# nekopanda/Amatsukaze

Measured on NVIDIA B200. Metric: 1920x1080i YV12 frames/sec (logo-eval + combing), higher is better.
Workload: dtype u8+f32

## Files before the change

### amatsukaze_b200/csrc/amtk_b200.cu

```cuda
#include "amtk_internal.h"
#include "logo_kernels.cuh"
#include "comb_kernels.cuh"
#include "comb_stream.cuh"
#include "comb_mma.cuh"
#include "scan_kernels.cuh"
#include <algorithm>
#include <cfloat>
#include <cmath>
#include <cstdlib>
#include <cstring>
#include <mutex>

extern "C" { static int logo_ensure_device(const amtk_logo* cl, amtk_ctx* ctx, bool need_tables); }

namespace amtk {

static thread_local std::string g_error;
static constexpr size_t kEvalSmemLimit = 226 * 1024;
void set_error(const std::string& msg) { g_error = msg; }
bool cuda_ok(cudaError_t e, const char* what) {
  if (e == cudaSuccess) return true;
  set_error(std::string("CUDA error: ") + cudaGetErrorString(e) + " in " + what);
  return false;
}
// ... 263 lines not shown
}

static bool roi_inside(const amtk::HostLogo& full, const amtk_clip* clip, int pitch_elems) {
  if (full.imgx < 0 || full.imgy < 0) return false;
  const long long last = (long long)full.imgx + full.w - 1 + (long long)(full.imgy + full.h - 1) * pitch_elems;
  const long long plane_elems = (long long)clip->pitch_y / clip->bytes_per_sample * clip->height;
  return full.imgx + full.w <= pitch_elems && last < plane_elems;
}

static int comb_thresholds_ok(const amtk_comb_params* p, int bytes_per_sample) {
  if (bytes_per_sample == 2) {
    const int all[6] = { p->th_move_y, p->th_shima_y, p->th_lshima_y, p->th_move_c, p->th_shima_c, p->th_lshima_c };
    for (int v : all) if (v < 1) { set_error("comb: thresholds must be >= 1"); return 0; }
    if (p->th_move_y > 32768 || p->th_move_c > 32768) { set_error("comb: th_move must be in [1,32768] for 16-bit samples"); return 0; }
    return 1;
  }
  const int m[2] = { p->th_move_y, p->th_move_c };
  const int s[4] = { p->th_shima_y, p->th_lshima_y, p->th_shima_c, p->th_lshima_c };
  for (int v : m) if (v < 1 || v > 128) { set_error("comb: th_move must be in [1,128]"); return 0; }
  for (int v : s) if (v < 1 || v > 2047) { set_error("comb: th_shima/th_lshima must be in [1,2047]"); return 0; }
  return 1;
}

struct CombVariant {
  int R, strip, stages, sync, TH, boxH, threads, smem;
  void (*kernel)(const CombArgs);
  void (*kernel16)(const CombArgs);
};
template <typename Cfg> static CombVariant make_variant() {
  return CombVariant{ Cfg::R, Cfg::STRIP, Cfg::STAGES, Cfg::SYNC, Cfg::TH, Cfg::BOXH, Cfg::THREADS, Cfg::SMEM, comb_tma_kernel<Cfg, 1>, nullptr };
}
template <typename Cfg> static CombVariant make_variant16() {
  return CombVariant{ Cfg::R, Cfg::STRIP, Cfg::STAGES, Cfg::SYNC, Cfg::TH, Cfg::BOXH, Cfg::THREADS, Cfg::SMEM, comb_tma_kernel<Cfg, 1>, comb_tma_kernel<Cfg, 2> };
}
static const CombVariant* comb_variants(int* n) {
  static const CombVariant v[] = {
    make_variant16<CombCfg<15, 8, 3, 0>>(), make_variant16<CombCfg<16, 8, 3, 0>>(), make_variant16<CombCfg<17, 8, 3, 0>>(),
    make_variant<CombCfg<17, 8, 2, 0>>(), make_variant<CombCfg<17, 8, 4, 0>>(), make_variant<CombCfg<17, 8, 3, 1>>(),
  };
  *n = (int)(sizeof(v) / sizeof(v[0]));
  return v;
}

static int pick_comb_R(int hY, int hC) {
  int best = 16; long long best_waste = -1;
  for (int R = 17; R >= 15; --R) {
    const int th = 8 * R;
    const long long waste = (long long)((hY + th - 1) / th) * th - hY + 2LL * (((hC + th - 1) / th) * th - hC) / 2;
    if (best_waste < 0 || waste < best_waste) { best_waste = waste; best = R; }
  }
  return best;
}

struct WsVariant { int R, stages, warps, bps, TH, boxH, smem; void (*kernel)(const WsArgs); };
template <typename Cfg> static WsVariant make_ws() { return WsVariant{ Cfg::R, Cfg::STAGES, Cfg::WARPS, Cfg::BPS, Cfg::TH, Cfg::BOXH, Cfg::SMEM, comb_ws_kernel<Cfg> }; }
static const WsVariant* ws_variants(int* n) {
  static const WsVariant v[] = { make_ws<WsCfg<17, 2>>(), make_ws<WsCfg<15, 2>>(), make_ws<WsCfg<16, 2>>(), make_ws<WsCfg<9, 2>>(), make_ws<WsCfg<15, 3>>(), make_ws<WsCfg<12, 2>>(), make_ws<WsCfg<10, 2>>(),
                                 make_ws<WsCfg<15, 2, 7>>(), make_ws<WsCfg<13, 2, 5>>(), make_ws<WsCfg<15, 2, 2>>(), make_ws<WsCfg<15, 3, 3>>(),
                                 make_ws<WsCfg<15, 2, 4, 2>>(), make_ws<WsCfg<16, 2, 4, 2>>(), make_ws<WsCfg<17, 2, 4, 2>>() };
  *n = (int)(sizeof(v) / sizeof(v[0]));
  return v;
}
static int pick_ws_R(int hY, int hC) {
  int best = 17; long long best_waste = -1;
  for (int R : { 17, 16, 15 }) {
    const int th = 4 * R;
    const long long waste = 2LL * ((long long)((hY + th - 1) / th) * th - hY) + 2LL * ((long long)((hC + th - 1) / th) * th - hC);
    if (best_waste < 0 || waste < best_waste) { best_waste = waste; best = R; }
  }
  return best;
}

static int launch_comb_ws(amtk_ctx* ctx, const amtk_clip* clip, const Window& win, int lo, int hi,
                          const amtk_comb_params* prm, int* dcounts, int out_row0) {
  const int hY = clip->height, hC = clip->height >> clip->log_uvy;
  const int wY = clip->width, wC = clip->width >> clip->log_uvx;
  const int R = ctx->knobs.comb_R ? ctx->knobs.comb_R : pick_ws_R(hY, hC);
  int nvar = 0; const WsVariant* vars = ws_variants(&nvar); const WsVariant* V = nullptr;
  const int bps = clip->bytes_per_sample;
  for (int i = 0; i < nvar; ++i) if (vars[i].R == R && vars[i].stages == ctx->knobs.comb_ws_stages && vars[i].warps == ctx->knobs.comb_ws_warps && vars[i].bps == bps) V = &vars[i];
  if (!V) AMTK_FAIL("comb: no warp-stream kernel variant for the requested AMTK_COMB_* settings");
  const int WW = V->warps;
  WsArgs args;
  memset(&args, 0, sizeof(args));
  const CUtensorMapL2promotion promo = ctx->knobs.comb_l2 == 0 ? CU_TENSOR_MAP_L2_PROMOTION_NONE : ctx->knobs.comb_l2 == 64 ? CU_TENSOR_MAP_L2_PROMOTION_L2_64B :
                                       ctx->knobs.comb_l2 == 256 ? CU_TENSOR_MAP_L2_PROMOTION_L2_256B : CU_TENSOR_MAP_L2_PROMOTION_L2_128B;
  for (int pl = 0; pl < 3; ++pl) {
    const long long off = pl == 0 ? 0 : (pl == 1 ? clip->off_u : clip->off_v);
    cuuint64_t gdim[3] = { (cuuint64_t)(pl ? wC : wY) * bps, (cuuint64_t)(pl ? hC : hY), (cuuint64_t)win.count };
    cuuint64_t gstr[2] = { (cuuint64_t)(pl ? clip->pitch_uv : clip->pitch_y), (cuuint64_t)clip->frame_stride };
    cuuint32_t box[3] = { (cuuint32_t)kWsTW, (cuuint32_t)V->boxH, 1u };
    cuuint32_t estr[3] = { 1u, 1u, 1u };
    if (ctx->encode_tiled(&args.map[pl], CU_TENSOR_MAP_DATA_TYPE_UINT8, 3, const_cast<uint8_t*>(win.dev_base) + off, gdim, gstr, box, estr,
                          CU_TENSOR_MAP_INTERLEAVE_NONE, CU_TENSOR_MAP_SWIZZLE_NONE, promo, CU_TENSOR_MAP_FLOAT_OOB_FILL_NONE) != CUDA_SUCCESS)
      AMTK_FAIL("cuTensorMapEncodeTiled failed");
  }
  const int remC = (wC * bps) % kWsTW;
  const long long uv_dist = clip->off_v - clip->off_u;
  const bool pair_uv = ctx->knobs.comb_merge_uv && remC > 0 && remC <= kWsTW / 2 && uv_dist > 0 && (uv_dist & 15) == 0;
  if (pair_uv) {
    cuuint64_t gdim[4] = { (cuuint64_t)wC * bps, 2u, (cuuint64_t)hC, (cuuint64_t)win.count };
    cuuint64_t gstr[3] = { (cuuint64_t)uv_dist, (cuuint64_t)clip->pitch_uv, (cuuint64_t)clip->frame_stride };
    cuuint32_t box[4] = { (cuuint32_t)(kWsTW / 2), 2u, (cuuint32_t)V->boxH, 1u };
    cuuint32_t estr[4] = { 1u, 1u, 1u, 1u };
    if (ctx->encode_tiled(&args.map_uv, CU_TENSOR_MAP_DATA_TYPE_UINT8, 4, const_cast<uint8_t*>(win.dev_base) + clip->off_u, gdim, gstr, box, estr,
                          CU_TENSOR_MAP_INTERLEAVE_NONE, CU_TENSOR_MAP_SWIZZLE_NONE, promo, CU_TENSOR_MAP_FLOAT_OOB_FILL_NONE) != CUDA_SUCCESS)
      AMTK_FAIL("cuTensorMapEncodeTiled(uv pair) failed");
  }
  const int tyY = (hY + V->TH - 1) / V->TH, tyC = (hC + V->TH - 1) / V->TH;
  int tile0 = 0, nc = 0;
  auto thresholds = [&](WsClass& C, bool chroma) {
    C.cls = chroma ? 1 : 0; C.H = chroma ? hC : hY;
    const int tM = chroma ? prm->th_move_c : prm->th_move_y, tS = chroma ? prm->th_shima_c : prm->th_shima_y, tL = chroma ? prm->th_lshima_c : prm->th_lshima_y;
    if (bps == 1) {
      C.thM = (unsigned)(0x80 - tM) * 0x01010101u;
      C.thS = (unsigned)tS * 0x00010001u;
      C.thL = (unsigned)tL * 0x00010001u;
    } else {
      C.thM = (unsigned)std::min(tM, 2047) * 0x00010001u;
      C.thS = (unsigned)(8192 + std::min(tS, 8191)) * 0x00010001u;
      C.thL = (unsigned)(8192 + std::min(tL, 8191)) * 0x00010001u;
    }
  };
  for (int pl = 0; pl < 3; ++pl) {
    WsClass& C = args.cl[nc];
    const int w = (pl ? wC : wY) * bps;
    C.kind = 0; C.map = pl; thresholds(C, pl != 0);
    C.tilesX = (pl && pair_uv) ? w / kWsTW : (w + kWsTW - 1) / kWsTW;
    C.tile0 = tile0; C.ntiles = C.tilesX * (pl ? tyC : tyY);
    if (C.ntiles == 0) continue;
    tile0 += C.ntiles; ++nc;
  }
  if (pair_uv) {
    WsClass& C = args.cl[nc];
    C.kind = 1; C.x0 = wC * bps - remC; C.tilesX = 1; thresholds(C, true);
    C.tile0 = tile0; C.ntiles = tyC; tile0 += C.ntiles; ++nc;
  }
  args.nclasses = nc;
  const int ntiles = tile0, nf = hi - lo;
  amtk_ctx::CombPlan& plan = ctx->plan;
  if (plan.occ_kernel != (const void*)V->kernel) {
    int occ = 0;
    AMTK_CUDA(cudaFuncSetAttribute(V->kernel, cudaFuncAttributeMaxDynamicSharedMemorySize, V->smem));
    AMTK_CUDA(cudaOccupancyMaxActiveBlocksPerMultiprocessor(&occ, V->kernel, 32 * WW, V->smem));
    if (occ < 1) AMTK_FAIL("comb kernel does not fit on an SM");
    plan.occ = occ; plan.occ_kernel = (const void*)V->kernel; plan.valid = false;
  }
  int occ = plan.occ;
  if (ctx->knobs.comb_ctas > 0) occ = std::min(occ, ctx->knobs.comb_ctas);
  const long long total = (long long)ntiles * nf;
  const int nwarps = ctx->sm_count * occ * WW;
  const int grid = (int)std::min<long long>((long long)ctx->sm_count * occ, (total + WW - 1) / WW);
  const int f0 = lo - win.first;
  if (!(plan.valid && plan.wY == wY && plan.hY == hY && plan.wC == wC && plan.hC == hC && plan.nf == nf && plan.f0 == f0 &&
        plan.R == V->R + 100 * bps && plan.item == ctx->knobs.comb_item + 1000 * ctx->knobs.comb_tail && plan.ctas == occ * WW)) {
    int big = ctx->knobs.comb_item > 0 ? ctx->knobs.comb_item : 64, small = std::max(4, big / 4);
    while (big > 8 && (long long)ntiles * (nf / big) < 6LL * nwarps) { big /= 2; small = std::max(4, big / 4); }
    const int tail_frames = std::min(nf, std::max(small, (int)(nf * 0.15)));
    const int head_frames = nf - tail_frames;
    const int tiny = ctx->knobs.comb_tail;
    const int end_frames = (tiny > 0 && tiny < small) ? std::min(tail_frames, std::max(tiny, (int)(nf * 0.04))) : 0;
    const int mid_end = nf - end_frames;
    std::vector<CombSegment> segs;
    segs.reserve((size_t)ntiles * (head_frames / big + tail_frames / small + (tiny > 0 ? end_frames / tiny : 0) + 3));
    for (int t = 0; t < ntiles; ++t)
      for (int f = 0; f < head_frames; f += big) segs.push_back(CombSegment{ t, f0 + f, f0 + std::min(head_frames, f + big) });
    for (int t = 0; t < ntiles; ++t)
      for (int f = head_frames; f < mid_end; f += small) segs.push_back(CombSegment{ t, f0 + f, f0 + std::min(mid_end, f + small) });
    for (int t = 0; t < ntiles; ++t)
      for (int f = mid_end; f < nf; f += tiny) segs.push_back(CombSegment{ t, f0 + f, f0 + std::min(nf, f + tiny) });
    const size_t seg_bytes = segs.size() * sizeof(CombSegment);
    plan.q_off = (seg_bytes + 255) & ~(size_t)255;
    plan.valid = false;
    if (!ensure(&plan.dev, &plan.cap, plan.q_off + 256)) return 0;
    AMTK_CUDA(cudaMemcpyAsync(plan.dev, segs.data(), seg_bytes, cudaMemcpyHostToDevice, ctx->stream));
    AMTK_CUDA(cudaStreamSynchronize(ctx->stream));
    plan.nitems = (int)segs.size();
    plan.wY = wY; plan.hY = hY; plan.wC = wC; plan.hC = hC; plan.nf = nf; plan.f0 = f0; plan.R = V->R + 100 * bps;
    plan.item = ctx->knobs.comb_item + 1000 * ctx->knobs.comb_tail; plan.ctas = occ * WW; plan.valid = true;
  }
  AMTK_CUDA(cudaMemsetAsync(reinterpret_cast<uint8_t*>(plan.dev) + plan.q_off, 0, 256, ctx->stream));
  args.segs = reinterpret_cast<const CombSegment*>(plan.dev);
  args.nitems = plan.nitems;
  args.queue = reinterpret_cast<int*>(reinterpret_cast<uint8_t*>(plan.dev) + plan.q_off);
  args.counts = dcounts;
  args.out_frame0 = out_row0 - win.first;
  AMTK_CUDA(cudaMemsetAsync(dcounts + (size_t)(lo - out_row0) * 12, 0, (size_t)nf * 12 * sizeof(int), ctx->stream));
  std::pair<cudaEvent_t, cudaEvent_t> ev{ nullptr, nullptr };
  if (ctx->timing) {
    if (!ctx->timing_pool.empty()) { ev = ctx->timing_pool.back(); ctx->timing_pool.pop_back(); }
    else { AMTK_CUDA(cudaEventCreate(&ev.first)); AMTK_CUDA(cudaEventCreate(&ev.second)); }
    AMTK_CUDA(cudaEventRecord(ev.first, ctx->stream));
  }
  args.prefetch = ctx->knobs.comb_ws_prefetch;
  if (ctx->want_side_mark) {
    AMTK_CUDA(cudaEventRecord(ctx->ev_side, ctx->stream));
    ctx->want_side_mark = false;
  }
  V->kernel<<<grid, 32 * WW, V->smem, ctx->stream>>>(args);
  AMTK_CUDA(cudaGetLastError());
  if (ctx->timing) { AMTK_CUDA(cudaEventRecord(ev.second, ctx->stream)); ctx->timing_events.push_back(ev); }
  ctx->launches += 1;
  return 1;
}

static int launch_comb_mma(amtk_ctx* ctx, const amtk_clip* clip, const Window& win, int lo, int hi,
                           const amtk_comb_params* prm, int* dcounts, int out_row0) {
  const int hY = clip->height, hC = clip->height >> clip->log_uvy;
  const int wY = clip->width, wC = clip->width >> clip->log_uvx;
  WsArgs args;
  memset(&args, 0, sizeof(args));
  const CUtensorMapL2promotion promo = ctx->knobs.comb_l2 == 0 ? CU_TENSOR_MAP_L2_PROMOTION_NONE : ctx->knobs.comb_l2 == 64 ? CU_TENSOR_MAP_L2_PROMOTION_L2_64B :
                                       ctx->knobs.comb_l2 == 256 ? CU_TENSOR_MAP_L2_PROMOTION_L2_256B : CU_TENSOR_MAP_L2_PROMOTION_L2_128B;
  for (int pl = 0; pl < 3; ++pl) {
    const long long off = pl == 0 ? 0 : (pl == 1 ? clip->off_u : clip->off_v);
    cuuint64_t gdim[3] = { (cuuint64_t)(pl ? wC : wY), (cuuint64_t)(pl ? hC : hY), (cuuint64_t)win.count };
    cuuint64_t gstr[2] = { (cuuint64_t)(pl ? clip->pitch_uv : clip->pitch_y), (cuuint64_t)clip->frame_stride };
    cuuint32_t box[3] = { (cuuint32_t)kMmTW, (cuuint32_t)kMmBoxH, 1u };
    cuuint32_t estr[3] = { 1u, 1u, 1u };
    if (ctx->encode_tiled(&args.map[pl], CU_TENSOR_MAP_DATA_TYPE_UINT8, 3, const_cast<uint8_t*>(win.dev_base) + off, gdim, gstr, box, estr,
                          CU_TENSOR_MAP_INTERLEAVE_NONE, CU_TENSOR_MAP_SWIZZLE_128B, promo, CU_TENSOR_MAP_FLOAT_OOB_FILL_NONE) != CUDA_SUCCESS)
      AMTK_FAIL("cuTensorMapEncodeTiled failed");
  }
  const int tyY = (hY + kMmTH - 1) / kMmTH, tyC = (hC + kMmTH - 1) / kMmTH;
  int tile0 = 0, nc = 0;
  for (int pl = 0; pl < 3; ++pl) {
    WsClass& C = args.cl[nc];
    const bool chroma = pl != 0;
    C.kind = 0; C.map = pl; C.cls = chroma ? 1 : 0; C.H = chroma ? hC : hY;
    C.thM = (unsigned)(0x80 - (chroma ? prm->th_move_c : prm->th_move_y)) * 0x01010101u;
    C.thS = (unsigned)(chroma ? prm->th_shima_c : prm->th_shima_y) * 0x00010001u;
// ... 244 lines not shown
  *out = nullptr;
  int n = 0;
  if (cudaGetDeviceCount(&n) != cudaSuccess || n == 0) { cudaGetLastError(); AMTK_FAIL("no CUDA device: this library has no CPU fallback"); }
  if (device < 0 || device >= n) AMTK_FAIL("amtk_ctx_create: bad device ordinal");
  int prev = 0; AMTK_CUDA(cudaGetDevice(&prev));
  AMTK_CUDA(cudaSetDevice(device));
  cudaDeviceProp prop; AMTK_CUDA(cudaGetDeviceProperties(&prop, device));
  if (prop.major != 10) { cudaSetDevice(prev); AMTK_FAIL("this build targets sm_100a (Blackwell B200) only"); }
  amtk_ctx* c = new amtk_ctx();
  c->device = device; c->sm_count = prop.multiProcessorCount;
  c->stream = reinterpret_cast<cudaStream_t>(cuda_stream); c->own_stream = false;
  bool ok = cuda_ok(cudaStreamCreateWithFlags(&c->copy_stream, cudaStreamNonBlocking), "cudaStreamCreate(copy)") &&
            cuda_ok(cudaStreamCreateWithFlags(&c->side_stream, cudaStreamNonBlocking), "cudaStreamCreate(side)") &&
            cuda_ok(cudaEventCreateWithFlags(&c->ev_side, cudaEventDisableTiming), "cudaEventCreate") &&
            cuda_ok(cudaEventCreateWithFlags(&c->ev_side_done, cudaEventDisableTiming), "cudaEventCreate") &&
            cuda_ok(cudaStreamCreateWithFlags(&c->side_stream2, cudaStreamNonBlocking), "cudaStreamCreate(side2)") &&
            cuda_ok(cudaEventCreateWithFlags(&c->ev_fork, cudaEventDisableTiming), "cudaEventCreate") &&
            cuda_ok(cudaEventCreateWithFlags(&c->ev_join1, cudaEventDisableTiming), "cudaEventCreate") &&
            cuda_ok(cudaEventCreateWithFlags(&c->ev_join2, cudaEventDisableTiming), "cudaEventCreate");
  for (int b = 0; b < 2 && ok; ++b) {
    ok = cuda_ok(cudaEventCreateWithFlags(&c->ev_copy[b], cudaEventDisableTiming), "cudaEventCreate") &&
         cuda_ok(cudaEventCreateWithFlags(&c->ev_done[b], cudaEventDisableTiming), "cudaEventCreate");
  }
  std::call_once(g_driver_once, [] {
    void* fn = nullptr; cudaDriverEntryPointQueryResult q;
    if (cudaGetDriverEntryPoint("cuTensorMapEncodeTiled", &fn, cudaEnableDefault, &q) == cudaSuccess && q == cudaDriverEntryPointSuccess)
      g_encode = reinterpret_cast<amtk_encode_tiled_fn>(fn);
    else cudaGetLastError();
  });
  c->encode_tiled = g_encode;
  if (const char* e = getenv("AMTK_COMB_STRIP")) c->knobs.comb_strip = atoi(e);
  if (const char* e = getenv("AMTK_COMB_STAGES")) c->knobs.comb_stages = atoi(e);
  if (const char* e = getenv("AMTK_COMB_R")) c->knobs.comb_R = atoi(e);
  if (const char* e = getenv("AMTK_COMB_CTAS")) c->knobs.comb_ctas = atoi(e);
  if (const char* e = getenv("AMTK_COMB_SYNC")) c->knobs.comb_sync = atoi(e);
  if (const char* e = getenv("AMTK_COMB_GENERIC")) c->knobs.comb_generic = atoi(e);
  if (const char* e = getenv("AMTK_COMB_MERGE_UV")) c->knobs.comb_merge_uv = atoi(e);
  if (const char* e = getenv("AMTK_COMB_PART")) c->knobs.comb_part = atoi(e);
  if (const char* e = getenv("AMTK_EVAL_WAVES")) c->knobs.eval_waves = std::max(1, atoi(e));
  if (const char* e = getenv("AMTK_COMB_L2")) c->knobs.comb_l2 = atoi(e);
  if (const char* e = getenv("AMTK_COMB_WS")) c->knobs.comb_ws = atoi(e);
  if (const char* e = getenv("AMTK_SCAN_LITE")) c->knobs.scan_lite = atoi(e);
  if (const char* e = getenv("AMTK_LITE_CTAS")) c->knobs.lite_ctas = std::max(1, atoi(e));
  if (const char* e = getenv("AMTK_COMB_WS_STAGES")) c->knobs.comb_ws_stages = atoi(e);
  if (const char* e = getenv("AMTK_COMB_ITEM")) c->knobs.comb_item = atoi(e);
  if (const char* e = getenv("AMTK_COMB_TAIL")) c->knobs.comb_tail = atoi(e);
  if (const char* e = getenv("AMTK_COMB_MMA")) c->knobs.comb_mma = atoi(e);
  if (const char* e = getenv("AMTK_COMB_WS10")) c->knobs.comb_ws10 = atoi(e);
  if (const char* e = getenv("AMTK_EVAL_CW")) c->knobs.eval_cw = atoi(e);
  if (const char* e = getenv("AMTK_EVAL_PAR")) c->knobs.eval_par = atoi(e);
  if (const char* e = getenv("AMTK_SCAN_OVERLAP")) c->knobs.scan_overlap = atoi(e);
  if (const char* e = getenv("AMTK_COMB_WS_WARPS")) c->knobs.comb_ws_warps = atoi(e);
  if (const char* e = getenv("AMTK_COMB_WS_PF")) c->knobs.comb_ws_prefetch = atoi(e);
  cudaSetDevice(prev);
  if (!ok) { amtk_ctx_destroy(c); return 0; }
  *out = c;
  return 1;
}

void amtk_ctx_destroy(amtk_ctx* c) {
  if (!c) return;
  int prev = 0; cudaGetDevice(&prev); cudaSetDevice(c->device);
  if (c->stream) cudaStreamSynchronize(c->stream);
  if (c->copy_stream) { cudaStreamSynchronize(c->copy_stream); cudaStreamDestroy(c->copy_stream); }
  if (c->side_stream) { cudaStreamSynchronize(c->side_stream); cudaStreamDestroy(c->side_stream); }
  if (c->ev_side) cudaEventDestroy(c->ev_side);
  if (c->ev_side_done) cudaEventDestroy(c->ev_side_done);
  if (c->side_stream2) { cudaStreamSynchronize(c->side_stream2); cudaStreamDestroy(c->side_stream2); }
  for (cudaEvent_t e : { c->ev_fork, c->ev_join1, c->ev_join2 }) if (e) cudaEventDestroy(e);
  for (int b = 0; b < 2; ++b) { if (c->ev_copy[b]) cudaEventDestroy(c->ev_copy[b]); if (c->ev_done[b]) cudaEventDestroy(c->ev_done[b]); if (c->stage[b]) cudaFree(c->stage[b]); }
  if (c->scratch) cudaFree(c->scratch);
  if (c->small) cudaFree(c->small);
  if (c->dout) cudaFree(c->dout);
  if (c->dout2) cudaFree(c->dout2);
  if (c->hout) cudaFreeHost(c->hout);
  if (c->plan.dev) cudaFree(c->plan.dev);
  for (auto* v : { &c->timing_events, &c->timing_pool }) for (auto& ev : *v) { cudaEventDestroy(ev.first); cudaEventDestroy(ev.second); }
  if (c->own_stream && c->stream) cudaStreamDestroy(c->stream);
  cudaSetDevice(prev);
  delete c;
}

int amtk_ctx_synchronize(amtk_ctx* c) {
  if (!c) AMTK_FAIL("null context");
  DevSelect ds(c); if (!ds.ok) return 0;
  AMTK_CUDA(cudaStreamSynchronize(c->stream));
  return 1;
}
int64_t amtk_ctx_launch_count(const amtk_ctx* c) { return c ? c->launches : 0; }
int64_t amtk_ctx_last_h2d_bytes(const amtk_ctx* c) { return c ? c->h2d_bytes_last : 0; }

int amtk_ctx_set_kernel_timing(amtk_ctx* c, int enable) {
  if (!c) AMTK_FAIL("null context");
  c->timing = enable != 0;
  return 1;
}

int amtk_ctx_get_kernel_timing(amtk_ctx* c, double* ms_total, int64_t* launches, int reset) {
  if (!c) AMTK_FAIL("null context");
  DevSelect ds(c); if (!ds.ok) return 0;
  AMTK_CUDA(cudaStreamSynchronize(c->stream));
  for (auto& ev : c->timing_events) {
    float ms = 0.0f;
    AMTK_CUDA(cudaEventElapsedTime(&ms, ev.first, ev.second));
    c->timing_ms += ms; c->timing_count += 1;
    c->timing_pool.push_back(ev);
// ... 728 lines not shown
```

### amatsukaze_b200/csrc/amtk_internal.h

```cpp
#pragma once
#include <cuda.h>
#include <cuda_runtime.h>
#include <cstdint>
#include <cstdio>
#include <mutex>
#include <string>
#include <vector>
#include "../../include/amtk_b200.h"
#include "logo_host.h"

typedef CUresult (*amtk_encode_tiled_fn)(CUtensorMap*, CUtensorMapDataType, cuuint32_t, void*, const cuuint64_t*,
                                         const cuuint64_t*, const cuuint32_t*, const cuuint32_t*, CUtensorMapInterleave,
                                         CUtensorMapSwizzle, CUtensorMapL2promotion, CUtensorMapFloatOOBfill);

namespace amtk {

void set_error(const std::string& msg);
bool cuda_ok(cudaError_t e, const char* what);

#define AMTK_CUDA(call)                                          \
  do {                                                           \
    if (!::amtk::cuda_ok((call), #call)) return 0;               \
  } while (0)
#define AMTK_FAIL(msg)                                           \
// ... 5 lines not shown
struct LogoDev {
  int w, h, count, countPad;
  float blackScore;
  const float* A;
  const float* B;
  const uint32_t* pix;
  const float* tapsT;
  const float2* scales;
};

}

struct amtk_ctx {
  mutable std::recursive_mutex mu;
  int device = 0;
  cudaStream_t stream = nullptr;
  bool own_stream = false;
  cudaStream_t copy_stream = nullptr;
  cudaStream_t side_stream = nullptr;
  cudaEvent_t ev_side = nullptr, ev_side_done = nullptr;
  cudaStream_t side_stream2 = nullptr;
  cudaEvent_t ev_fork = nullptr, ev_join1 = nullptr, ev_join2 = nullptr;
  size_t scratch_off = 0;
  cudaEvent_t ev_copy[2] = { nullptr, nullptr };
  cudaEvent_t ev_done[2] = { nullptr, nullptr };
  int sm_count = 0;
  int64_t launches = 0;
  long long h2d_bytes_last = 0;
  void* scratch = nullptr; size_t scratch_bytes = 0;
  void* stage[2] = { nullptr, nullptr }; size_t stage_bytes = 0;
  void* small = nullptr; size_t small_bytes = 0;
  void* dout = nullptr; size_t dout_bytes = 0;
  void* dout2 = nullptr; size_t dout2_bytes = 0;
  std::vector<std::pair<const void*, int>> smem_attr;
  void* hout = nullptr; void* hout_dev = nullptr;
  amtk_encode_tiled_fn encode_tiled = nullptr;
  bool want_side_mark = false;
  struct Knobs {
    int eval_waves = 1;
    int eval_cw = 1;
    int eval_par = 1;
    int scan_overlap = 0;
    int comb_generic = 0;
    int comb_merge_uv = 1;
    int comb_part = -1;
    int comb_strip = 8, comb_stages = 3, comb_R = 0, comb_ctas = 0, comb_sync = 0, comb_l2 = 64;
    int comb_item = 0;
    int comb_tail = 4;
    int comb_ws_stages = 2;
    int comb_mma = 0;
    int comb_ws10 = 1;
    int comb_ws_warps = 4;
    int comb_ws_prefetch = 0;
    int lite_ctas = 5;
    int scan_lite = 0;
    int comb_ws = 1;
  } knobs;
  struct CombPlan {
    bool valid = false;
    int wY = 0, hY = 0, wC = 0, hC = 0, nf = 0, f0 = 0, R = 0, item = 0, ctas = 0;
    void* dev = nullptr; size_t cap = 0;
    int nitems = 0; size_t q_off = 0;
    int occ = 0; const void* occ_kernel = nullptr;
  } plan;
  bool timing = false;
  std::vector<std::pair<cudaEvent_t, cudaEvent_t>> timing_events;
  std::vector<std::pair<cudaEvent_t, cudaEvent_t>> timing_pool;
  double timing_ms = 0.0; int64_t timing_count = 0;
};

struct amtk_logo {
  int device = -1;
  amtk::HostLogo host;
  float* dA = nullptr; float* dB = nullptr;
  float* dAU = nullptr; float* dBU = nullptr; float* dAV = nullptr; float* dBV = nullptr;
  uint32_t* dPix = nullptr; float* dTapsT = nullptr; float2* dScales = nullptr;
  int countPad = 0;
  bool has_mask = false;
  bool tables_uploaded = false;
  std::mutex mu;
};

struct amtk_scan {
  amtk_ctx* ctx = nullptr;
  int device = 0;
  int scanw = 0, scanh = 0, logUVx = 1, logUVy = 1, thy = 0;
  int nvalid = 0;
  unsigned long long* dSums = nullptr;
  unsigned long long* dBg = nullptr;
  size_t npix = 0;
};
```

### amatsukaze_b200/csrc/comb_stream.cuh

```cuda
#pragma once
#include <cuda_fp16.h>
#include "amtk_internal.h"
#include "tma_utils.cuh"
#include "comb_kernels.cuh"

namespace amtk {

constexpr int kWsTW = 128;
constexpr int kWsRuns = 4;
constexpr int kWsWarps = 4;

template <int R_, int STAGES_, int WARPS_ = kWsWarps, int BPS_ = 1>
struct WsCfg {
  static constexpr int R = R_, STAGES = STAGES_, WARPS = WARPS_;
  static constexpr int BPS = BPS_;
  static constexpr int TH = kWsRuns * R;
  static constexpr int BOXH = TH + 4;
  static constexpr int STAGE_BYTES = kWsTW * BOXH;
  static constexpr int RING_BYTES = STAGES * STAGE_BYTES;
  static constexpr int SMEM = WARPS * RING_BYTES + 128;
  static constexpr int FIT = (227 * 1024) / (SMEM + 1024 + 8 * WARPS * STAGES + 8);
  static constexpr int MIN_CTAS = FIT >= 4 ? 4 : FIT >= 3 ? 3 : FIT >= 2 ? 2 : 1;
};

struct WsClass {
  int tile0, ntiles;
  int kind;
  int tilesX;
  int map;
  int x0;
  int H;
  int cls;
  unsigned thM, thS, thL;
};
constexpr int kWsMaxClasses = 4;
struct WsArgs {
  CUtensorMap map[3];
  CUtensorMap map_uv;
  WsClass cl[kWsMaxClasses];
  int nclasses;
  const CombSegment* segs;
  int nitems;
  int* queue;
  int* counts;
  int out_frame0;
  int prefetch;
};

__device__ __forceinline__ void tma_load_4d(void* smem_dst, const CUtensorMap* map, uint64_t* bar, int c0, int c1, int c2, int c3) {
  asm volatile(
      "cp.async.bulk.tensor.4d.shared::cluster.global.mbarrier::complete_tx::bytes [%0], [%1, {%3, %4, %5, %6}], [%2];"
      ::"r"(smem_u32(smem_dst)), "l"(map), "r"(smem_u32(bar)), "r"(c0), "r"(c1), "r"(c2), "r"(c3)
      : "memory");
}

__device__ __forceinline__ void tma_prefetch_3d(const CUtensorMap* map, int c0, int c1, int c2) {
  asm volatile("cp.async.bulk.prefetch.tensor.3d.L2.global.tile [%0, {%1, %2, %3}];" ::"l"(map), "r"(c0), "r"(c1), "r"(c2) : "memory");
}
__device__ __forceinline__ void tma_prefetch_4d(const CUtensorMap* map, int c0, int c1, int c2, int c3) {
  asm volatile("cp.async.bulk.prefetch.tensor.4d.L2.global.tile [%0, {%1, %2, %3, %4}];" ::"l"(map), "r"(c0), "r"(c1), "r"(c2), "r"(c3) : "memory");
}

#ifndef AMTK_WS_RELOAD_PREV
#define AMTK_WS_RELOAD_PREV 1
#endif
constexpr bool kWsReloadPrev = AMTK_WS_RELOAD_PREV != 0;
#ifndef AMTK_WS_L_VIA_IDP
#define AMTK_WS_L_VIA_IDP 0
#endif
// ... 167 lines not shown
  W4 h2 = w4(*reinterpret_cast<const uint4*>(cur + 2 * PITCH));
  W4 h3 = w4(*reinterpret_cast<const uint4*>(cur + 3 * PITCH));
#pragma unroll
  for (int j = 0; j < R; ++j) {
    const W4 h4 = w4(*reinterpret_cast<const uint4*>(cur + (j + 4) * PITCH));
    const W4 pv = w4(P[j]);
    const int f = j & 1;
    uint32_t mM[4];
#pragma unroll
    for (int q = 0; q < 4; ++q)
      mM[q] = __hge2_mask(__habs2(__hsub2(*reinterpret_cast<const __half2*>(&h2.v[q]), *reinterpret_cast<const __half2*>(&pv.v[q]))), thM);
    c.M[f] = c.M[f] - (mM[0] + mM[1]) - (mM[2] + mM[3]);
    if (kWsReloadPrev) P[j] = lds128(cur + (j + 2) * PITCH); else P[j] = make_uint4(h2.v[0], h2.v[1], h2.v[2], h2.v[3]);
    ws_row_masks10(h0, h1, h2, h3, h4, thS, thL, c.S[f], c.L[f]);
    h0 = h1; h1 = h2; h2 = h3; h3 = h4;
  }
  return c;
}

template <int PITCH>
__device__ __noinline__ void ws_fixup10(const uint8_t* cur, uint32_t rows, uint32_t mine, uint32_t thS_bits, uint32_t thL_bits, WsCounts& c) {
  const __half2 thS = *reinterpret_cast<const __half2*>(&thS_bits);
  const __half2 thL = *reinterpret_cast<const __half2*>(&thL_bits);
  for (uint32_t m = rows; m; m &= m - 1) {
    const int j = __ffs(m) - 1;
    if (!((mine >> j) & 1u)) continue;
    const uint8_t* p = cur + j * PITCH;
    uint32_t dS = 0u, dL = 0u;
    ws_row_masks10(w4(*reinterpret_cast<const uint4*>(p)), w4(*reinterpret_cast<const uint4*>(p + PITCH)), w4(*reinterpret_cast<const uint4*>(p + 2 * PITCH)),
                   w4(*reinterpret_cast<const uint4*>(p + 3 * PITCH)), w4(*reinterpret_cast<const uint4*>(p + 4 * PITCH)), thS, thL, dS, dL);
    c.S[j & 1] -= dS; c.L[j & 1] -= dL;
  }
}

template <int PITCH>
__device__ __noinline__ void ws_fixup(const uint8_t* cur, uint32_t rows, uint32_t mine, uint32_t thS_bits, uint32_t thL_bits, WsCounts& c) {
  const __half2 thS = *reinterpret_cast<const __half2*>(&thS_bits);
  const __half2 thL = *reinterpret_cast<const __half2*>(&thL_bits);
  for (uint32_t m = rows; m; m &= m - 1) {
    const int j = __ffs(m) - 1;
    if (!((mine >> j) & 1u)) continue;
    const uint8_t* p = cur + j * PITCH;
    const H8 h0 = bytes16_to_half(*reinterpret_cast<const uint4*>(p));
    const H8 h1 = bytes16_to_half(*reinterpret_cast<const uint4*>(p + PITCH));
    const H8 h2 = bytes16_to_half(*reinterpret_cast<const uint4*>(p + 2 * PITCH));
    const H8 h3 = bytes16_to_half(*reinterpret_cast<const uint4*>(p + 3 * PITCH));
    const H8 h4 = bytes16_to_half(*reinterpret_cast<const uint4*>(p + 4 * PITCH));
    uint32_t dS = 0u, dL = 0u;
    ws_row_masks(h0, h1, h2, h3, h4, thS, thL, dS, dL);
    c.S[j & 1] -= dS; c.L[j & 1] -= dL;
  }
}

template <typename Cfg>
__global__ void __launch_bounds__(32 * Cfg::WARPS, Cfg::MIN_CTAS) comb_ws_kernel(const __grid_constant__ WsArgs a) {
  constexpr int S = Cfg::STAGES, R = Cfg::R;
  extern __shared__ uint8_t smem_raw[];
  __shared__ __align__(8) uint64_t full_bars[Cfg::WARPS][S];
  const int lane = threadIdx.x & 31, warp = threadIdx.x >> 5;
  uint8_t* tiles = smem_raw + ((128u - (smem_u32(smem_raw) & 127u)) & 127u) + warp * Cfg::RING_BYTES;
  uint64_t* full_bar = full_bars[warp];
  if (lane == 0) {
#pragma unroll
    for (int s = 0; s < S; ++s) mbar_init(&full_bar[s], 1);
    asm volatile("fence.mbarrier_init.release.cluster;" ::: "memory");
  }
  __syncwarp();
  uint32_t gload = 0;
  const int strip = lane & 7, run = lane >> 3;
  const int lane_off = (run * R) * kWsTW + strip * 16;
  for (;;) {
    int item = 0;
    if (lane == 0) item = atomicAdd(a.queue, 1);
    item = __shfl_sync(0xFFFFFFFFu, item, 0);
    if (item >= a.nitems) break;
    const CombSegment seg = a.segs[item];
    int ci = 0;
#pragma unroll
    for (int k = 1; k < kWsMaxClasses; ++k) if (k < a.nclasses && seg.tile >= a.cl[k].tile0) ci = k;
    const WsClass& C = a.cl[ci];
    const int lt = seg.tile - C.tile0;
    const int ty = lt / C.tilesX, tx = lt - ty * C.tilesX;
    const int y0 = ty * Cfg::TH;
    const int y_first = y0 + run * R;
    const int nf = seg.fend - seg.fbegin;
    const int nloads = nf + 1;
    const int fprev = seg.fbegin > 0 ? seg.fbegin - 1 : seg.fbegin;

    auto issue_at = [&](int j, int st) {
      const int fr = (j == 0) ? fprev : seg.fbegin + j - 1;
      mbar_expect_tx(&full_bar[st], Cfg::STAGE_BYTES);
      uint8_t* dst = tiles + st * Cfg::STAGE_BYTES;
      if (C.kind == 0) tma_load_3d(dst, &a.map[C.map], &full_bar[st], tx * kWsTW, y0 - 2, fr);
      else tma_load_4d(dst, &a.map_uv, &full_bar[st], C.x0, 0, y0 - 2, fr);
    };
    auto prefetch_at = [&](int j) {
      const int fr = seg.fbegin + j - 1;
      if (C.kind == 0) tma_prefetch_3d(&a.map[C.map], tx * kWsTW, y0 - 2, fr);
      else tma_prefetch_4d(&a.map_uv, C.x0, 0, y0 - 2, fr);
    };
    const int pf = a.prefetch;
    if (lane == 0) {
      const int pro = nloads < S ? nloads : S;
      for (int j = 0; j < pro; ++j) issue_at(j, (int)((gload + (uint32_t)j) % S));
      for (int j = S; j < S + pf && j < nloads; ++j) prefetch_at(j);
    }
    uint32_t fix_mine = 0u;
    if (y_first < 2) fix_mine |= (1u << (2 - y_first)) - 1u;
    {
      const int lo_j = max(C.H - 2 - y_first, 0), hi_j = min(C.H + 2 - y_first, R);
      if (hi_j > lo_j) fix_mine |= ((1u << hi_j) - 1u) & ~((1u << lo_j) - 1u);
    }
    const uint32_t fix_rows = __reduce_or_sync(0xFFFFFFFFu, fix_mine);
    const int flip = y_first & 1;
    const uint32_t kM = C.thM, tS = C.thS, tL = C.thL;
    int* const crow = a.counts + C.cls * 6 + lane + ((long long)seg.fbegin - 1 - a.out_frame0) * 12;

    int st = (int)(gload % S);
    uint32_t ph = (gload / S) & 1u;
    mbar_wait(&full_bar[st], ph);
    uint4 P[R];
    {
      const uint8_t* l0 = tiles + st * Cfg::STAGE_BYTES + lane_off;
#pragma unroll
      for (int j = 0; j < R; ++j) P[j] = *reinterpret_cast<const uint4*>(l0 + (j + 2) * kWsTW);
      __syncwarp();
      if (lane == 0 && S < nloads) issue_at(S, st);
      if (lane == 0 && pf > 0 && S + pf < nloads) prefetch_at(S + pf);
    }
    for (int k = 1; k <= nf; ++k) {
      if (++st == S) { st = 0; ph ^= 1u; }
      mbar_wait(&full_bar[st], ph);
      const uint8_t* cur = tiles + st * Cfg::STAGE_BYTES + lane_off;
      WsCounts c = Cfg::BPS == 2 ? ws_rows10<R, kWsTW>(cur, P, kM, tS, tL)
                                 : (AMTK_WS_SP ? ws_rows_sp<R, kWsTW>(cur, P, kM, tS, tL) : ws_rows<R, kWsTW>(cur, P, kM, tS, tL));
      if (fix_rows) {
        if (Cfg::BPS == 2) ws_fixup10<kWsTW>(cur, fix_rows, fix_mine, tS, tL, c); else ws_fixup<kWsTW>(cur, fix_rows, fix_mine, tS, tL, c);
        __syncwarp();
      }
      const uint32_t s0 = flip ? c.S[1] : c.S[0], s1 = flip ? c.S[0] : c.S[1];
      const uint32_t l0 = flip ? c.L[1] : c.L[0], l1 = flip ? c.L[0] : c.L[1];
      const uint32_t m0 = flip ? c.M[1] : c.M[0], m1 = flip ? c.M[0] : c.M[1];
      const uint32_t rM0 = __reduce_add_sync(0xFFFFFFFFu, m0), rS0 = __reduce_add_sync(0xFFFFFFFFu, s0), rL0 = __reduce_add_sync(0xFFFFFFFFu, l0);
      const uint32_t rM1 = __reduce_add_sync(0xFFFFFFFFu, m1), rS1 = __reduce_add_sync(0xFFFFFFFFu, s1), rL1 = __reduce_add_sync(0xFFFFFFFFu, l1);
      __syncwarp();
      if (lane == 0 && (k + S) < nloads) issue_at(k + S, st);
      if (lane == 0 && pf > 0 && (k + S + pf) < nloads) prefetch_at(k + S + pf);
      if (lane < 6) {
        const int fld = lane >= 3, met = lane - 3 * fld;
        uint32_t v = met == 0 ? (fld ? rM1 : rM0) : met == 1 ? (fld ? rS1 : rS0) : (fld ? rL1 : rL0);
        v = (met == 0 && Cfg::BPS == 1) ? (v >> 7) : (met == 2 && kWsLviaIdp && Cfg::BPS == 1) ? v / 510u : decode_pair(v);
        if (v) atomicAdd(crow + (size_t)k * 12, (int)v);
      }
    }
    gload += (uint32_t)nloads;
  }
}

}
// ... 1 lines not shown
```

Measured before the change: 1.370 million.

## Add tensor-core mma.sync path for 8-bit combing stencil in warp-stream kernel

Adds a new warp-stream combing variant for 8-bit samples. It loads tile rows with transposed ldmatrix, converts bytes to fp16 and evaluates the vertical 5-tap stencil as an m16n8k16 HMMA against a banded weight matrix, replacing per-row SIMD byte arithmetic. Thresholds are re-encoded as half values and edge rows are handled by a separate fp16 fixup, with results reduced per warp. The path is on by default through a new HMMA knob and uses R=8 with 64-row tiles. This changes tile geometry and register pressure, and the fp16 rounding could shift threshold edge cases.

```diff
diff --git a/amatsukaze_b200/csrc/amtk_b200.cu b/amatsukaze_b200/csrc/amtk_b200.cu
--- a/amatsukaze_b200/csrc/amtk_b200.cu
+++ b/amatsukaze_b200/csrc/amtk_b200.cu
@@ -339,12 +339,13 @@
   return best;
 }
 
-struct WsVariant { int R, stages, warps, bps, TH, boxH, smem; void (*kernel)(const WsArgs); };
-template <typename Cfg> static WsVariant make_ws() { return WsVariant{ Cfg::R, Cfg::STAGES, Cfg::WARPS, Cfg::BPS, Cfg::TH, Cfg::BOXH, Cfg::SMEM, comb_ws_kernel<Cfg> }; }
+struct WsVariant { int R, stages, warps, bps, mma, TH, boxH, smem; void (*kernel)(const WsArgs); };
+template <typename Cfg> static WsVariant make_ws() { return WsVariant{ Cfg::R, Cfg::STAGES, Cfg::WARPS, Cfg::BPS, Cfg::MMA, Cfg::TH, Cfg::BOXH, Cfg::SMEM, comb_ws_kernel<Cfg> }; }
 static const WsVariant* ws_variants(int* n) {
   static const WsVariant v[] = { make_ws<WsCfg<17, 2>>(), make_ws<WsCfg<15, 2>>(), make_ws<WsCfg<16, 2>>(), make_ws<WsCfg<9, 2>>(), make_ws<WsCfg<15, 3>>(), make_ws<WsCfg<12, 2>>(), make_ws<WsCfg<10, 2>>(),
                                  make_ws<WsCfg<15, 2, 7>>(), make_ws<WsCfg<13, 2, 5>>(), make_ws<WsCfg<15, 2, 2>>(), make_ws<WsCfg<15, 3, 3>>(),
-                                 make_ws<WsCfg<15, 2, 4, 2>>(), make_ws<WsCfg<16, 2, 4, 2>>(), make_ws<WsCfg<17, 2, 4, 2>>() };
+                                 make_ws<WsCfg<15, 2, 4, 2>>(), make_ws<WsCfg<16, 2, 4, 2>>(), make_ws<WsCfg<17, 2, 4, 2>>(),
+                                 make_ws<WsCfg<8, 2, 4, 1, 1>>() };
   *n = (int)(sizeof(v) / sizeof(v[0]));
   return v;
 }
@@ -362,10 +363,12 @@
                           const amtk_comb_params* prm, int* dcounts, int out_row0) {
   const int hY = clip->height, hC = clip->height >> clip->log_uvy;
   const int wY = clip->width, wC = clip->width >> clip->log_uvx;
-  const int R = ctx->knobs.comb_R ? ctx->knobs.comb_R : pick_ws_R(hY, hC);
+  const int bps = clip->bytes_per_sample;
+  const int mma = bps == 1 && ctx->knobs.comb_ws_hmma ? 1 : 0;
+  const int R = mma ? 8 : ctx->knobs.comb_R ? ctx->knobs.comb_R : pick_ws_R(hY, hC);
   int nvar = 0; const WsVariant* vars = ws_variants(&nvar); const WsVariant* V = nullptr;
-  const int bps = clip->bytes_per_sample;
-  for (int i = 0; i < nvar; ++i) if (vars[i].R == R && vars[i].stages == ctx->knobs.comb_ws_stages && vars[i].warps == ctx->knobs.comb_ws_warps && vars[i].bps == bps) V = &vars[i];
+  for (int i = 0; i < nvar; ++i)
+    if (vars[i].R == R && vars[i].stages == ctx->knobs.comb_ws_stages && vars[i].warps == ctx->knobs.comb_ws_warps && vars[i].bps == bps && vars[i].mma == mma) V = &vars[i];
   if (!V) AMTK_FAIL("comb: no warp-stream kernel variant for the requested AMTK_COMB_* settings");
   const int WW = V->warps;
   WsArgs args;
@@ -399,7 +402,12 @@
   auto thresholds = [&](WsClass& C, bool chroma) {
     C.cls = chroma ? 1 : 0; C.H = chroma ? hC : hY;
     const int tM = chroma ? prm->th_move_c : prm->th_move_y, tS = chroma ? prm->th_shima_c : prm->th_shima_y, tL = chroma ? prm->th_lshima_c : prm->th_lshima_y;
-    if (bps == 1) {
+    if (mma) {
+      C.thM = (unsigned)(0x80 - tM) * 0x01010101u;
+      const __half hs = __float2half_rn((float)std::min(tS, 2047) / 2048.0f), hl = __float2half_rn((float)(1 - std::min(tL, 2047)));
+      C.thS = (unsigned)__half_as_ushort(hs) * 0x00010001u;
+      C.thL = (unsigned)__half_as_ushort(hl) * 0x00010001u;
+    } else if (bps == 1) {
       C.thM = (unsigned)(0x80 - tM) * 0x01010101u;
       C.thS = (unsigned)tS * 0x00010001u;
       C.thL = (unsigned)tL * 0x00010001u;
@@ -440,7 +448,7 @@
   const int grid = (int)std::min<long long>((long long)ctx->sm_count * occ, (total + WW - 1) / WW);
   const int f0 = lo - win.first;
   if (!(plan.valid && plan.wY == wY && plan.hY == hY && plan.wC == wC && plan.hC == hC && plan.nf == nf && plan.f0 == f0 &&
-        plan.R == V->R + 100 * bps && plan.item == ctx->knobs.comb_item + 1000 * ctx->knobs.comb_tail && plan.ctas == occ * WW)) {
+        plan.R == V->R + 100 * bps + 1000 * mma && plan.item == ctx->knobs.comb_item + 1000 * ctx->knobs.comb_tail && plan.ctas == occ * WW)) {
     int big = ctx->knobs.comb_item > 0 ? ctx->knobs.comb_item : 64, small = std::max(4, big / 4);
     while (big > 8 && (long long)ntiles * (nf / big) < 6LL * nwarps) { big /= 2; small = std::max(4, big / 4); }
     const int tail_frames = std::min(nf, std::max(small, (int)(nf * 0.15)));
@@ -463,7 +471,7 @@
     AMTK_CUDA(cudaMemcpyAsync(plan.dev, segs.data(), seg_bytes, cudaMemcpyHostToDevice, ctx->stream));
     AMTK_CUDA(cudaStreamSynchronize(ctx->stream));
     plan.nitems = (int)segs.size();
-    plan.wY = wY; plan.hY = hY; plan.wC = wC; plan.hC = hC; plan.nf = nf; plan.f0 = f0; plan.R = V->R + 100 * bps;
+    plan.wY = wY; plan.hY = hY; plan.wC = wC; plan.hC = hC; plan.nf = nf; plan.f0 = f0; plan.R = V->R + 100 * bps + 1000 * mma;
     plan.item = ctx->knobs.comb_item + 1000 * ctx->knobs.comb_tail; plan.ctas = occ * WW; plan.valid = true;
   }
   AMTK_CUDA(cudaMemsetAsync(reinterpret_cast<uint8_t*>(plan.dev) + plan.q_off, 0, 256, ctx->stream));
@@ -814,6 +822,7 @@
   if (const char* e = getenv("AMTK_SCAN_OVERLAP")) c->knobs.scan_overlap = atoi(e);
   if (const char* e = getenv("AMTK_COMB_WS_WARPS")) c->knobs.comb_ws_warps = atoi(e);
   if (const char* e = getenv("AMTK_COMB_WS_PF")) c->knobs.comb_ws_prefetch = atoi(e);
+  if (const char* e = getenv("AMTK_COMB_WS_HMMA")) c->knobs.comb_ws_hmma = atoi(e);
   cudaSetDevice(prev);
   if (!ok) { amtk_ctx_destroy(c); return 0; }
   *out = c;
diff --git a/amatsukaze_b200/csrc/amtk_internal.h b/amatsukaze_b200/csrc/amtk_internal.h
--- a/amatsukaze_b200/csrc/amtk_internal.h
+++ b/amatsukaze_b200/csrc/amtk_internal.h
@@ -81,6 +81,7 @@
     int comb_ws10 = 1;
     int comb_ws_warps = 4;
     int comb_ws_prefetch = 0;
+    int comb_ws_hmma = 1;
     int lite_ctas = 5;
     int scan_lite = 0;
     int comb_ws = 1;
diff --git a/amatsukaze_b200/csrc/comb_stream.cuh b/amatsukaze_b200/csrc/comb_stream.cuh
--- a/amatsukaze_b200/csrc/comb_stream.cuh
+++ b/amatsukaze_b200/csrc/comb_stream.cuh
@@ -10,11 +10,13 @@
 constexpr int kWsRuns = 4;
 constexpr int kWsWarps = 4;
 
-template <int R_, int STAGES_, int WARPS_ = kWsWarps, int BPS_ = 1>
+template <int R_, int STAGES_, int WARPS_ = kWsWarps, int BPS_ = 1, int MMA_ = 0>
 struct WsCfg {
   static constexpr int R = R_, STAGES = STAGES_, WARPS = WARPS_;
   static constexpr int BPS = BPS_;
-  static constexpr int TH = kWsRuns * R;
+  static constexpr bool MMA = MMA_ != 0;
+  static_assert(!MMA || BPS == 1, "the mma.sync body is for 8-bit samples");
+  static constexpr int TH = MMA ? 8 * R : kWsRuns * R;
   static constexpr int BOXH = TH + 4;
   static constexpr int STAGE_BYTES = kWsTW * BOXH;
   static constexpr int RING_BYTES = STAGES * STAGE_BYTES;
@@ -288,6 +290,107 @@
   }
 }
 
+struct WsMmaCounts { uint32_t S, L, M; };
+constexpr uint32_t kWsMmaOne = 0x3C003C00u;
+constexpr uint32_t kWsMmaBias = 0x64006400u;
+
+__device__ __forceinline__ void ldsm_x4_t(uint32_t* r, const uint8_t* p) {
+  asm volatile("ldmatrix.sync.aligned.m8n8.x4.trans.shared.b16 {%0, %1, %2, %3}, [%4];"
+               : "=r"(r[0]), "=r"(r[1]), "=r"(r[2]), "=r"(r[3]) : "r"(smem_u32(p)));
+}
+__device__ __forceinline__ void mma_band(const uint32_t a0, const uint32_t a1, const uint32_t a2, const uint32_t a3,
+                                         const uint32_t b0, const uint32_t b1, uint32_t& d0, uint32_t& d1) {
+  asm("mma.sync.aligned.m16n8k16.row.col.f16.f16.f16.f16 {%0, %1}, {%2, %3, %4, %5}, {%6, %7}, {%8, %8};"
+      : "=r"(d0), "=r"(d1) : "r"(a0), "r"(a1), "r"(a2), "r"(a3), "r"(b0), "r"(b1), "r"(0u));
+}
+
+__device__ __forceinline__ void ws_mma_band(const int lane, uint32_t& b0, uint32_t& b1) {
+  const int g = lane >> 2, t = lane & 3;
+  auto w = [&](int i) { const int k = i - g; return k < 0 || k > 4 ? 0.0f : (k == 2 ? 4.0f : (k & 1) ? -3.0f : 1.0f) * 8192.0f; };
+  auto pair = [&](int i) { __half2 h = __floats2half2_rn(w(i), w(i + 2)); return *reinterpret_cast<uint32_t*>(&h); };
+  b0 = t < 2 ? pair(t & 1) : 0u;
+  b1 = pair((t < 2 ? 8 : 4) + (t & 1));
+}
+
+template <int NB, int PITCH>
+__device__ __forceinline__ WsMmaCounts ws_rows_mma(const uint8_t* __restrict__ slot, uint32_t (&P)[NB + 1][8],
+                                                   const uint32_t off_pro, const uint32_t off_new, const uint32_t b0, const uint32_t b1,
+                                                   const uint32_t kM, const uint32_t thS_bits, const uint32_t thL_bits) {
+  const __half2 thS = *reinterpret_cast<const __half2*>(&thS_bits);
+  const __half2 nthL = *reinterpret_cast<const __half2*>(&thL_bits);
+  const __half2 k2048 = __float2half2_rn(2048.0f);
+  const bool t01 = (threadIdx.x & 3) < 2;
+  const uint32_t wPro = t01 ? 0x01010000u : 0u;
+  const uint32_t wLast = t01 ? 0x00000101u : 0x01010101u;
+  uint32_t accS = 0u, accM = 0u, accLb = kWsMmaBias;
+  uint32_t lo[8][2], hi[8][2];
+  auto moved = [&](const uint32_t (&raw)[8], uint32_t (&prev)[8], const uint32_t w) {
+#pragma unroll
+    for (int i = 0; i < 8; ++i) { accM = __dp4a(bytes_ge(__vabsdiffu4(raw[i], prev[i]), kM), w, accM); prev[i] = raw[i]; }
+  };
+  auto pairs = [&](const uint32_t (&raw)[8], uint32_t (&dst)[8][2]) {
+#pragma unroll
+    for (int i = 0; i < 8; ++i) { dst[i][0] = __byte_perm(raw[i], 0u, 0x4240); dst[i][1] = __byte_perm(raw[i], 0u, 0x4341); }
+  };
+  {
+    uint32_t raw[8];
+    ldsm_x4_t(raw, slot + off_pro); ldsm_x4_t(raw + 4, slot + off_pro + 64);
+    moved(raw, P[0], wPro);
+    pairs(raw, lo);
+  }
+#pragma unroll
+  for (int b = 0; b < NB; ++b) {
+    uint32_t raw[8];
+    ldsm_x4_t(raw, slot + off_new + 8 * b * PITCH); ldsm_x4_t(raw + 4, slot + off_new + 8 * b * PITCH + 64);
+    moved(raw, P[b + 1], b == NB - 1 ? wLast : 0x01010101u);
+    if (b & 1) pairs(raw, lo); else pairs(raw, hi);
+    const uint32_t B0 = (b & 1) ? b1 : b0, B1 = (b & 1) ? b0 : b1;
+    __half2 accL = *reinterpret_cast<const __half2*>(&accLb);
+#pragma unroll
+    for (int i = 0; i < 8; ++i) {
+      uint32_t d[2];
+      mma_band(lo[i][0], lo[i][1], hi[i][0], hi[i][1], B0, B1, d[0], d[1]);
+#pragma unroll
+      for (int e = 0; e < 2; ++e) {
+        const __half2 r = __habs2(*reinterpret_cast<const __half2*>(&d[e]));
+        accS -= __hge2_mask(r, thS);
+        accL = __hadd2(accL, __hfma2_sat(r, k2048, nthL));
+      }
+    }
+    accLb = *reinterpret_cast<const uint32_t*>(&accL);
+  }
+  return WsMmaCounts{ accS, accLb - kWsMmaBias, accM };
+}
+
+template <int PITCH>
+__device__ __noinline__ void ws_fixup_mma(const uint8_t* slot, uint64_t rows, int lane, uint32_t thS_bits, uint32_t thL_bits, WsMmaCounts& c) {
+  const __half2 thS = *reinterpret_cast<const __half2*>(&thS_bits);
+  const __half2 nthL = *reinterpret_cast<const __half2*>(&thL_bits);
+  const __half2 k4 = __float2half2_rn(4.0f), km3 = __float2half2_rn(-3.0f), k8192 = __float2half2_rn(8192.0f), k2048 = __float2half2_rn(2048.0f);
+  const __half2 one = __float2half2_rn(1.0f);
+  for (uint64_t m = rows; m; m &= m - 1) {
+    const int j = __ffsll((long long)m) - 1;
+    const uint8_t* p = slot + j * PITCH + lane * 4;
+    __half2 h[5][2];
+#pragma unroll
+    for (int k = 0; k < 5; ++k) {
+      const uint32_t w = *reinterpret_cast<const uint32_t*>(p + k * PITCH);
+      uint32_t a = __byte_perm(w, 0, 0x4140), b = __byte_perm(w, 0, 0x4342);
+      h[k][0] = *reinterpret_cast<__half2*>(&a); h[k][1] = *reinterpret_cast<__half2*>(&b);
+    }
+    uint32_t nS = 0u, nL = 0u;
+#pragma unroll
+    for (int q = 0; q < 2; ++q) {
+      __half2 t = __hfma2(k4, h[2][q], __hadd2(h[0][q], h[4][q]));
+      const __half2 r = __habs2(__hmul2(__hfma2(km3, __hadd2(h[1][q], h[3][q]), t), k8192));
+      nS += __popc(__hge2_mask(r, thS)) >> 4;
+      nL += __popc(__hge2_mask(__hfma2_sat(r, k2048, nthL), one)) >> 4;
+    }
+    c.S += nS * ((j & 1) ? 0xFFFF0000u : 0x0000FFFFu);
+    c.L -= nL << ((j & 1) * 16);
+  }
+}
+
 template <typename Cfg>
 __global__ void __launch_bounds__(32 * Cfg::WARPS, Cfg::MIN_CTAS) comb_ws_kernel(const __grid_constant__ WsArgs a) {
   constexpr int S = Cfg::STAGES, R = Cfg::R;
@@ -305,6 +408,11 @@
   uint32_t gload = 0;
   const int strip = lane & 7, run = lane >> 3;
   const int lane_off = (run * R) * kWsTW + strip * 16;
+  const int rho = lane & 7, rt = rho >> 1;
+  const uint32_t mm_pro = ((rt & 1) + 2 * (rho & 1)) * kWsTW + (lane >> 3) * 16;
+  const uint32_t mm_new = ((rt < 2 ? 8 : 4) + (rt & 1) + 2 * (rho & 1)) * kWsTW + (lane >> 3) * 16;
+  uint32_t mm_b0 = 0u, mm_b1 = 0u;
+  if (Cfg::MMA) ws_mma_band(lane, mm_b0, mm_b1);
   for (;;) {
     int item = 0;
     if (lane == 0) item = atomicAdd(a.queue, 1);
@@ -341,6 +449,53 @@
       for (int j = 0; j < pro; ++j) issue_at(j, (int)((gload + (uint32_t)j) % S));
       for (int j = S; j < S + pf && j < nloads; ++j) prefetch_at(j);
     }
+    if constexpr (Cfg::MMA) {
+      uint64_t fix_rows = 0u;
+      if (y0 < 2) fix_rows |= (1ull << (2 - y0)) - 1u;
+      {
+        const int lo_j = max(C.H - 2 - y0, 0), hi_j = min(C.H + 2 - y0, Cfg::TH);
+        if (hi_j > lo_j) fix_rows |= (hi_j >= 64 ? ~0ull : (1ull << hi_j) - 1u) & ~((1ull << lo_j) - 1u);
+      }
+      const uint32_t kM = C.thM, tS = C.thS, tL = C.thL;
+      int* const crow = a.counts + C.cls * 6 + lane + ((long long)seg.fbegin - 1 - a.out_frame0) * 12;
+      int st = (int)(gload % S);
+      uint32_t ph = (gload / S) & 1u;
+      mbar_wait(&full_bar[st], ph);
+      uint32_t P[R + 1][8];
+      {
+        const uint8_t* l0 = tiles + st * Cfg::STAGE_BYTES;
+        ldsm_x4_t(P[0], l0 + mm_pro); ldsm_x4_t(P[0] + 4, l0 + mm_pro + 64);
+#pragma unroll
+        for (int b = 0; b < R; ++b) { ldsm_x4_t(P[b + 1], l0 + mm_new + 8 * b * kWsTW); ldsm_x4_t(P[b + 1] + 4, l0 + mm_new + 8 * b * kWsTW + 64); }
+        __syncwarp();
+        if (lane == 0 && S < nloads) issue_at(S, st);
+        if (lane == 0 && pf > 0 && S + pf < nloads) prefetch_at(S + pf);
+      }
+      for (int k = 1; k <= nf; ++k) {
+        if (++st == S) { st = 0; ph ^= 1u; }
+        mbar_wait(&full_bar[st], ph);
+        const uint8_t* slot = tiles + st * Cfg::STAGE_BYTES;
+        WsMmaCounts c = ws_rows_mma<R, kWsTW>(slot, P, mm_pro, mm_new, mm_b0, mm_b1, kM, tS, tL);
+        if (fix_rows) {
+          ws_fixup_mma<kWsTW>(slot, fix_rows, lane, tS, tL, c);
+          __syncwarp();
+        }
+        const uint32_t odd = lane & 1;
+        const uint32_t rM0 = __reduce_add_sync(0xFFFFFFFFu, odd ? 0u : c.M), rM1 = __reduce_add_sync(0xFFFFFFFFu, odd ? c.M : 0u);
+        const uint32_t rS = __reduce_add_sync(0xFFFFFFFFu, c.S), rL = __reduce_add_sync(0xFFFFFFFFu, c.L);
+        __syncwarp();
+        if (lane == 0 && (k + S) < nloads) issue_at(k + S, st);
+        if (lane == 0 && pf > 0 && (k + S + pf) < nloads) prefetch_at(k + S + pf);
+        if (lane < 6) {
+          const int fld = lane >= 3, met = lane - 3 * fld;
+          const uint32_t s0 = rS & 0xFFFFu, s1 = ((rS >> 16) + s0) & 0xFFFFu;
+          const uint32_t v = met == 0 ? (fld ? rM1 : rM0) >> 7 : met == 1 ? (fld ? s1 : s0) : (fld ? rL >> 16 : rL & 0xFFFFu);
+          if (v) atomicAdd(crow + (size_t)k * 12, (int)v);
+        }
+      }
+      gload += (uint32_t)nloads;
+      continue;
+    }
     uint32_t fix_mine = 0u;
     if (y_first < 2) fix_mine |= (1u << (2 - y_first)) - 1u;
     {
```

Result: slower. 994,100 (median of 6 runs) (-27.4%).
